# ChalmersPhotonicsLab/QAMpy

Hardware: AMD Instinct MI355X
Metric: equalised MSym/s (2-pol, 2 SPS) (higher is better)
Workload: dtype f32

## Files before the change

### qampy_amd/csrc/train_pit.h

```cpp
#pragma once
#include <atomic>
#include <chrono>
#include <vector>
#include "train_impl.h"
#include "train_seg.h"

namespace qh {

typedef qh_pit_report PitCtrl;

constexpr double PIT_CONTRACT = 0.2;
constexpr int PIT_PROBE = 128;
constexpr int PIT_SEEDWIN = 512;
constexpr int PIT_MAXSEG = 65536;

__host__ __device__ inline int pit_symmetry(int method)
{
    switch (method) {
    case QH_M_CMA: case QH_M_SGNCMA: case QH_M_RDE: return 0;
    case QH_M_CMA2: return 2;
    default: return 4;
    }
}

// ... 763 lines not shown
                        const float c = __builtin_amdgcn_rsqf(1.f + t * t);
                        g = float4{c, t * c, apq.x * rmag, apq.y * rmag};
                    }
                }
                grot[tid] = g; gpair[tid] = ix;
                glog[((size_t)sweep * (m - 1) + r) * npair + tid] = g;
            }
            __syncthreads();
#pragma unroll
            for (int k = 0; k < NB; k++) {
                if (k >= nbt) break;
                const int I = bI[k], J = bJ[k];
                const int2 pi = gpair[I], pj = gpair[J];
                const float4 gi = grot[I], gj = grot[J];
                const bool qi = pi.y < n, qj = pj.y < n;
                const Zf z{0.f, 0.f};
                const Zf a_pr = src[pi.x * ld + pj.x], a_ps = qj ? src[pi.x * ld + pj.y] : z;
                const Zf a_qr = qi ? src[pi.y * ld + pj.x] : z, a_qs = (qi && qj) ? src[pi.y * ld + pj.y] : z;
                const Zf ejc{gj.z, -gj.w};
                const Zf ps_e = cmulf(ejc, a_ps), qs_e = cmulf(ejc, a_qs);
                const Zf t_pr{gj.x * a_pr.x - gj.y * ps_e.x, gj.x * a_pr.y - gj.y * ps_e.y}, t_ps{gj.y * a_pr.x + gj.x * ps_e.x, gj.y * a_pr.y + gj.x * ps_e.y};
                const Zf t_qr{gj.x * a_qr.x - gj.y * qs_e.x, gj.x * a_qr.y - gj.y * qs_e.y}, t_qs{gj.y * a_qr.x + gj.x * qs_e.x, gj.y * a_qr.y + gj.x * qs_e.y};
                const Zf ei{gi.z, gi.w};
                const Zf qr_e = cmulf(ei, t_qr), qs_e2 = cmulf(ei, t_qs);
                const Zf n_pr{gi.x * t_pr.x - gi.y * qr_e.x, gi.x * t_pr.y - gi.y * qr_e.y}, n_ps{gi.x * t_ps.x - gi.y * qs_e2.x, gi.x * t_ps.y - gi.y * qs_e2.y};
                const Zf n_qr{gi.y * t_pr.x + gi.x * qr_e.x, gi.y * t_pr.y + gi.x * qr_e.y}, n_qs{gi.y * t_ps.x + gi.x * qs_e2.x, gi.y * t_ps.y + gi.x * qs_e2.y};
                dst[pi.x * ld + pj.x] = n_pr;
                if (qj) dst[pi.x * ld + pj.y] = n_ps;
                if (qi) dst[pi.y * ld + pj.x] = n_qr;
                if (qi && qj) dst[pi.y * ld + pj.y] = n_qs;
                if (I != J) {
                    dst[pj.x * ld + pi.x] = Zf{n_pr.x, -n_pr.y};
                    if (qj) dst[pj.y * ld + pi.x] = Zf{n_ps.x, -n_ps.y};
                    if (qi) dst[pj.x * ld + pi.y] = Zf{n_qr.x, -n_qr.y};
                    if (qi && qj) dst[pj.y * ld + pi.y] = Zf{n_qs.x, -n_qs.y};
                }
            }
            __syncthreads();
            Zf *t = src; src = dst; dst = t;
        }
    }
    for (int k = tid; k < n; k += 1024) lam[k] = (double)src[k * ld + k].x;
}

constexpr int PIT_JV_CH = 27;
static __global__ void __launch_bounds__(64) pit_jacobi_v_kernel(const float4 *glog, int n, int nsweep, Zf *Vout)
{
    QH_WAVE_FIRST();
    __shared__ Zf row[PIT_EIGMAX + 2];
    __shared__ float4 gch[PIT_JV_CH * (PIT_EIGMAX / 2 + 1)];
    const int lane = threadIdx.x, i = blockIdx.x;
    const int m = (n + 1) & ~1, npair = m / 2;
    for (int k = lane; k < n + 2; k += 64) row[k] = Zf{k == i ? 1.f : 0.f, 0.f};
    const int nround = nsweep * (m - 1);
    for (int r0 = 0; r0 < nround; r0 += PIT_JV_CH) {
        const int nr = nround - r0 < PIT_JV_CH ? nround - r0 : PIT_JV_CH;
        __syncthreads();
        for (int e = lane; e < nr * npair; e += 64) gch[e] = glog[(size_t)r0 * npair + e];
        __syncthreads();
        for (int rr = 0; rr < nr; rr++) {
            const int r = (r0 + rr) % (m - 1);
            if (lane < npair) {
                int pa, pb;
                if (lane == 0) { pa = m - 1; pb = r; }
                else {
                    pa = r + lane; if (pa >= m - 1) pa -= m - 1;
                    pb = r - lane; if (pb < 0) pb += m - 1;
                }
                const int p = pa < pb ? pa : pb, q = pa < pb ? pb : pa;
                if (q < n) {
                    const float4 g = gch[rr * npair + lane];
                    const Zf up = row[p];
                    const Zf xqe = cmulf(Zf{g.z, -g.w}, row[q]);
                    row[p] = Zf{g.x * up.x - g.y * xqe.x, g.x * up.y - g.y * xqe.y};
                    row[q] = Zf{g.y * up.x + g.x * xqe.x, g.y * up.y + g.x * xqe.y};
                }
            }
            __builtin_amdgcn_fence(__ATOMIC_RELEASE, "wavefront");
        }
    }
    for (int k = lane; k < n; k += 64) { Vout[(size_t)i * n + k] = row[k]; Vout[(size_t)n * n + (size_t)k * n + i] = row[k]; }
}

constexpr int PIT_GT = 16, PIT_GC = PIT_GT / 8;
template <typename R> struct PitFuse {
    Cx<R> *X, *Y;
    const double *theta;
    const int64_t *modes_dev;
    int nmodes, nsel;
    float damp = 1.f;
    const Cx<R> *T2 = nullptr;
    float2 *Out2 = nullptr;
};
template <typename R, bool CONJT>
__global__ void __launch_bounds__(256) pit_cgemm_kernel(const Zf *A2, const Zf *B, Zf *C, int n, int ncol, const PitCtrl *c, PitFuse<R> fz)
{
    QH_WAVE_FIRST();
    if (c->done) return;
    extern __shared__ __attribute__((aligned(16))) char pit_smem[];
    Zf *As = reinterpret_cast<Zf *>(pit_smem);
    Zf *Bs = As + (size_t)PIT_EIGMAX * PIT_EIGMAX;
    const int tx = threadIdx.x & 7, ty = threadIdx.x >> 3;
    const int col0 = blockIdx.x * PIT_GT;
    const size_t wset = (size_t)fz.nmodes * n;
    for (int e = threadIdx.x; e < PIT_EIGMAX * n; e += 256) {
        const int k = e / PIT_EIGMAX, m = e - k * PIT_EIGMAX;
        Zf v{0.f, 0.f};
        if (m < n) { v = A2[(size_t)k * n + m]; if (CONJT) v.y = -v.y; }
        As[e] = v;
    }
    if (CONJT) {
        for (int e = threadIdx.x; e < n * PIT_GT; e += 256) {
            const int cc = e / n, k = e - cc * n, col = col0 + cc;
            Zf v{0.f, 0.f};
            if (col < ncol) {
                const int s = col / fz.nsel, j = col - s * fz.nsel;
                if (s > 0) {
                    const size_t ro = (size_t)fz.modes_dev[j] * n;
                    const Cx<R> b = fz.Y[(size_t)(s - 1) * wset + ro + k], a = fz.X[(size_t)s * wset + ro + k];
                    const double pr = fz.theta[2 * (size_t)(col - fz.nsel)], pi = fz.theta[2 * (size_t)(col - fz.nsel) + 1];
                    const double qr = fz.theta[2 * (size_t)col], qi = fz.theta[2 * (size_t)col + 1];
                    v = Zf{(float)((pr * b.re - pi * b.im) - (qr * a.re - qi * a.im)), (float)((pr * b.im + pi * b.re) - (qr * a.im + qi * a.re))};
                }
            }
            Bs[k * PIT_GT + cc] = v;
        }
    } else {
        for (int e = threadIdx.x; e < n * PIT_GT; e += 256) {
            const int k = e / PIT_GT, cc = e - k * PIT_GT;
            Bs[e] = col0 + cc < ncol ? B[(size_t)k * ncol + col0 + cc] : Zf{0.f, 0.f};
        }
    }
    __syncthreads();
    constexpr int RU = PIT_EIGMAX / 32;
    Zf acc[RU][PIT_GC];
#pragma unroll
    for (int u = 0; u < RU; u++)
#pragma unroll
        for (int v = 0; v < PIT_GC; v++) acc[u][v] = Zf{0.f, 0.f};
    for (int k = 0; k < n; k++) {
        Zf b[PIT_GC], a[RU];
#pragma unroll
        for (int v = 0; v < PIT_GC; v++) b[v] = Bs[k * PIT_GT + PIT_GC * tx + v];
#pragma unroll
        for (int u = 0; u < RU; u++) a[u] = As[k * PIT_EIGMAX + ty + 32 * u];
#pragma unroll
        for (int u = 0; u < RU; u++)
#pragma unroll
            for (int v = 0; v < PIT_GC; v++) {
                acc[u][v].x += a[u].x * b[v].x - a[u].y * b[v].y;
                acc[u][v].y += a[u].x * b[v].y + a[u].y * b[v].x;
            }
    }
    if (CONJT) {
#pragma unroll
        for (int u = 0; u < RU; u++) {
            const int m = ty + 32 * u;
            if (m < n)
#pragma unroll
                for (int v = 0; v < PIT_GC; v++)
                    if (col0 + PIT_GC * tx + v < ncol) C[(size_t)m * ncol + col0 + PIT_GC * tx + v] = acc[u][v];
        }
    } else {
#pragma unroll
        for (int v = 0; v < PIT_GC; v++) {
            const int col = col0 + PIT_GC * tx + v;
            if (col >= ncol) continue;
            const int s = col / fz.nsel, j = col - s * fz.nsel;
            const size_t base = (size_t)s * wset + (size_t)fz.modes_dev[j] * n;
            const double qr = fz.theta[2 * (size_t)col], qi = fz.theta[2 * (size_t)col + 1];
#pragma unroll
            for (int u = 0; u < RU; u++) {
                const int m = ty + 32 * u;
                if (m < n) {
                    const Cx<R> x = fz.X[base + m];
// ... 220 lines not shown
        for (int cb = 0; cb < PIT_MC; cb += NCW * nw) {
            Zf tmp[NCW][2];
#pragma unroll
            for (int q = 0; q < NCW; q++) {
                const int cc = cb + wave + nw * q, col = col0 + cc;
                tmp[q][0] = Zf{0.f, 0.f}; tmp[q][1] = Zf{0.f, 0.f};
                if (cc < PIT_MC && col < ncol) {
                    const int s = col / fz.nsel, j = col - s * fz.nsel;
                    const Cx<R> *src = T + (size_t)s * wset + (size_t)fz.modes_dev[j] * n;
                    if (lane < n) { const Cx<R> t = src[lane]; tmp[q][0] = Zf{(float)t.re, (float)t.im}; }
                    if (lane + 64 < n) { const Cx<R> t = src[lane + 64]; tmp[q][1] = Zf{(float)t.re, (float)t.im}; }
                }
            }
#pragma unroll
            for (int q = 0; q < NCW; q++) {
                const int cc = cb + wave + nw * q;
                if (cc < PIT_MC) {
                    if (lane < np) Bs[lane * PIT_MBP + cc] = tmp[q][0];
                    if (lane + 64 < np) Bs[(lane + 64) * PIT_MBP + cc] = tmp[q][1];
                }
            }
        }
    } else {
        const int cc = tid & 15, k0 = tid >> 4, kstep = nt >> 4;
        const bool okc = col0 + cc < ncol;
        for (int kb = 0; kb < np; kb += 8 * kstep) {
            Zf tmp[8];
#pragma unroll
            for (int q = 0; q < 8; q++) {
                const int k = kb + k0 + kstep * q;
                tmp[q] = (okc && k < n) ? D[(size_t)k * ncol + col0 + cc] : Zf{0.f, 0.f};
            }
#pragma unroll
            for (int q = 0; q < 8; q++) {
                const int k = kb + k0 + kstep * q;
                if (k < np) Bs[k * PIT_MBP + cc] = tmp[q];
            }
        }
    }
    const bool pre = MODE == 1 && NCW * nw >= PIT_MC;
    Cx<R> xv[MODE == 1 ? NCW : 1][2];
    double th[MODE == 1 ? NCW : 1][2];
    if (pre) {
#pragma unroll
        for (int q = 0; q < NCW; q++) {
            const int cc = wave + nw * q, col = col0 + cc;
            xv[q][0] = Cx<R>{0, 0}; xv[q][1] = Cx<R>{0, 0}; th[q][0] = 1; th[q][1] = 0;
            if (cc < PIT_MC && col < ncol) {
                const int s = col / fz.nsel, j = col - s * fz.nsel;
                const size_t base = (size_t)s * wset + (size_t)fz.modes_dev[j] * n;
                th[q][0] = fz.theta[2 * (size_t)col]; th[q][1] = fz.theta[2 * (size_t)col + 1];
                if (lane < n) xv[q][0] = fz.X[base + lane];
                if (lane + 64 < n) xv[q][1] = fz.X[base + lane + 64];
            }
        }
    }
    __syncthreads();
    pit_f4 rr = {0.f, 0.f, 0.f, 0.f}, ii = rr, im = rr;
    const Zf *bp = Bs + (lane >> 4) * PIT_MBP + (lane & 15);
    for (int k0 = 0; k0 < np; k0 += 4 * PF) {
#pragma unroll
        for (int i = 0; i < PF; i++) {
            const int k = k0 + 4 * i;
            if (k < np) {
                Zf a = abuf[i];
                abuf[i] = lda(k + 4 * PF);
                if (MODE == 0) a.y = -a.y;
                const Zf b = bp[(size_t)k * PIT_MBP];
                rr = __builtin_amdgcn_mfma_f32_16x16x4f32(a.x, b.x, rr, 0, 0, 0);
                ii = __builtin_amdgcn_mfma_f32_16x16x4f32(a.y, b.y, ii, 0, 0, 0);
                im = __builtin_amdgcn_mfma_f32_16x16x4f32(a.x, b.y, im, 0, 0, 0);
                im = __builtin_amdgcn_mfma_f32_16x16x4f32(a.y, b.x, im, 0, 0, 0);
            }
        }
    }
    const int cl = lane & 15;
    if (MODE == 0) {
        const int col = col0 + cl;
#pragma unroll
        for (int q = 0; q < 4; q++) {
            const int m = 16 * wave + 4 * (lane >> 4) + q;
            if (m < n && col < ncol) Out[(size_t)m * ncol + col] = Zf{rr[q] - ii[q], im[q]};
        }
    } else {
#pragma unroll
        for (int q = 0; q < 4; q++) {
            const int m = 16 * wave + 4 * (lane >> 4) + q;
            Ct[cl * (PIT_EIGMAX + 1) + m] = Zf{rr[q] - ii[q], im[q]};
        }
        __syncthreads();
        for (int cb = 0; cb < PIT_MC; cb += NCW * nw) {
#pragma unroll
            for (int q = 0; q < NCW; q++) {
                const int cc = cb + wave + nw * q, col = col0 + cc;
                if (cc < PIT_MC && col < ncol) {
                    const int s = col / fz.nsel, j = col - s * fz.nsel;
                    const size_t base = (size_t)s * wset + (size_t)fz.modes_dev[j] * n;
                    const double qr = pre ? th[q][0] : fz.theta[2 * (size_t)col], qi = pre ? th[q][1] : fz.theta[2 * (size_t)col + 1];
#pragma unroll
                    for (int h = 0; h < 2; h++) {
                        const int m = lane + 64 * h;
                        if (m < n) {
                            const Cx<R> x = pre ? xv[q][h] : fz.X[base + m];
                            const Zf d = Ct[cc * (PIT_EIGMAX + 1) + m];
                            const Cx<R> w{(R)(qr * x.re - qi * x.im + fz.damp * d.x), (R)(qr * x.im + qi * x.re + fz.damp * d.y)};
                            fz.X[base + m] = w;
                            fz.Y[base + m] = w;
                        }
                    }
                }
            }
        }
    }
}

static __global__ void __launch_bounds__(256) pit_bound_kernel(const Zf *Xe, const Zf *Ye, const Zf *Yprev, const double *lam, int n, int S, int nsel, int sym,
                                                              const PitCtrl *c, double *dfc, double *pw, double *gph, float4 *ualpha = nullptr)
{
    QH_WAVE_FIRST();
    if (c->done) return;
    const int lane = threadIdx.x & 63, bi = blockIdx.x * 4 + (threadIdx.x >> 6);
    const int nb = (S - 1) * nsel, ncol = S * nsel;
    if (bi >= nb + nsel) return;
    const bool result_probe = bi >= nb;
    const int j = result_probe ? bi - nb : bi % nsel;
    const int sb = result_probe ? S - 1 : bi / nsel;
    const Zf *pa = result_probe ? (c->passes == 0 ? Xe + (size_t)(S - 1) * nsel + j : Yprev + j) : Xe + (size_t)(sb + 1) * nsel + j;
    const size_t sa = (result_probe && c->passes != 0) ? (size_t)nsel : (size_t)ncol;
    const Zf *pb = Ye + (size_t)sb * nsel + j;
    Zf av[(PIT_EIGMAX + 63) / 64], bv[(PIT_EIGMAX + 63) / 64];
    float lv[(PIT_EIGMAX + 63) / 64];
    double A = 0, B = 0, Cr = 0, Ci = 0;
#pragma unroll
    for (int q = 0; q < (PIT_EIGMAX + 63) / 64; q++) {
        const int k = lane + 64 * q;
        av[q] = Zf{0.f, 0.f}; bv[q] = Zf{0.f, 0.f}; lv[q] = 0.f;
        if (k < n) {
            av[q] = pa[(size_t)k * sa]; bv[q] = pb[(size_t)k * ncol];
            const float l = (float)lam[k];
            lv[q] = l > 0.f ? l : 0.f;
        }
        A += (double)lv[q] * ((double)av[q].x * av[q].x + (double)av[q].y * av[q].y);
        B += (double)lv[q] * ((double)bv[q].x * bv[q].x + (double)bv[q].y * bv[q].y);
        Cr += (double)lv[q] * ((double)bv[q].x * av[q].x + (double)bv[q].y * av[q].y);
        Ci += (double)lv[q] * ((double)bv[q].y * av[q].x - (double)bv[q].x * av[q].y);
    }
    for (int o = 32; o > 0; o >>= 1) { A += __shfl_xor(A, o); B += __shfl_xor(B, o); Cr += __shfl_xor(Cr, o); Ci += __shfl_xor(Ci, o); }
    double gr = 1, gi = 0;
    if (sym == 0) {
        const double pr = sqrt(Cr * Cr + Ci * Ci);
        if (pr > 0) { gr = Cr / pr; gi = Ci / pr; }
    } else if (sym == 4 || sym == 2 || sym == 1) {
        if (sym == 4 && fabs(Ci) > fabs(Cr)) { gr = 0; gi = Ci >= 0 ? 1 : -1; }
        else if (sym == 1) gr = 1;
        else gr = Cr >= 0 ? 1 : -1;
    } else {
        const double step = 6.283185307179586 / sym;
        const double kk = rint(atan2(Ci, Cr) / step) * step;
        gr = cos(kk); gi = sin(kk);
    }
    double d2 = 0;
    const float grf = (float)gr, gif = (float)gi;
#pragma unroll
    for (int q = 0; q < (PIT_EIGMAX + 63) / 64; q++) {
        const float dr = bv[q].x - (grf * av[q].x - gif * av[q].y), di = bv[q].y - (grf * av[q].y + gif * av[q].x);
        d2 += (double)lv[q] * ((double)dr * dr + (double)di * di);
    }
    for (int o = 32; o > 0; o >>= 1) d2 += __shfl_xor(d2, o);
    if (ualpha && !result_probe) {
        float nn = 0.f, ar = 0.f, ai = 0.f;
#pragma unroll
        for (int q = 0; q < (PIT_EIGMAX + 63) / 64; q++) {
            const float dr = bv[q].x - (grf * av[q].x - gif * av[q].y), di = bv[q].y - (grf * av[q].y + gif * av[q].x);
            const float ur = lv[q] * bv[q].x, ui = lv[q] * bv[q].y;
            nn += ur * ur + ui * ui;
            ar += ur * dr + ui * di;
            ai += ur * di - ui * dr;
        }
        for (int o = 32; o > 0; o >>= 1) { nn += __shfl_xor(nn, o); ar += __shfl_xor(ar, o); ai += __shfl_xor(ai, o); }
        const float inv = nn > 0.f ? rsqrtf(nn) : 0.f;
        if (lane == 0) ualpha[bi] = float4{ar * inv, ai * inv, inv, 0.f};
    }
    if (lane == 0) {
        if (!result_probe) { gph[2 * (size_t)bi] = gr; gph[2 * (size_t)bi + 1] = gi; pw[bi] = B; }
        dfc[bi] = (A == A && B == B) ? sqrt(d2 / (B > 1e-300 ? B : 1e-300)) : 1e30;
    }
}

constexpr int PIT_RT = 1024;
template <typename R>
__global__ void __launch_bounds__(PIT_RT) pit_recur_eig_kernel(Zf *Xe, const Zf *Ye, Zf *D, const double *theta, const double *lam, int nsel, int S, int64_t T, const R *mu,
                                                               double beta, const PitCtrl *c, const float *Msum = nullptr, float damp = 1.f,
                                                               const float4 *ualpha = nullptr, const float2 *uq = nullptr)
{
    QH_WAVE_FIRST();
    if (c->done) return;
    __shared__ float4 aff[2 * PIT_RT];
    const int k = blockIdx.x, j = blockIdx.y;
    const int ncol = S * nsel;
    Zf *row = D + (size_t)k * ncol + j, *xr = Xe + (size_t)k * ncol + j;
    const Zf *yr = Ye + (size_t)k * ncol + j;
    double a = (double)*mu * c->gain * (double)T * lam[k];
    if (a < 0) a = 0;
    const float coef = c->corr_on ? (float)exp(-a * (1 + beta * a)) : 0.f;
    const float gl = (float)(c->gain * lam[k] > 0 ? c->gain * lam[k] : 0.0), betaf = (float)beta;
    const bool corr = c->corr_on != 0;
    auto cf = [&](int s) -> float {
        if (!Msum) return coef;
        const float as = gl * Msum[(size_t)s * nsel + j];
        return corr ? __expf(-as * (1.f + betaf * as)) : 0.f;
    };
    const int len = (S + PIT_RT - 1) / PIT_RT;
    const int s0 = threadIdx.x * len, s1 = s0 + len < S ? s0 + len : S;
    auto th = [&](int s) { return Zf{(float)theta[2 * ((size_t)s * nsel + j)], (float)theta[2 * ((size_t)s * nsel + j) + 1]}; };
    auto scan_op = [](float4 e, float4 l) { return float4{l.x * e.x, l.x * e.y + l.y, l.x * e.z + l.z, 0.f}; };
    if (len <= 4) {
        Zf y[4], x[4], t[5], r[4];
        t[0] = s0 > 0 && s0 < S ? th(s0 - 1) : Zf{1.f, 0.f};
#pragma unroll
        for (int q = 0; q < 4; q++) {
            const int s = s0 + q;
            const bool ok = s < s1;
            y[q] = (ok && s > 0) ? yr[(size_t)(s - 1) * nsel] : Zf{0.f, 0.f};
            x[q] = ok ? xr[(size_t)s * nsel] : Zf{0.f, 0.f};
            t[q + 1] = ok ? th(s) : Zf{1.f, 0.f};
        }
        Zf run{0.f, 0.f};
        float cq[4], clen = 1.f;
        float4 ua[4];
        float2 qq[4];
        const float lk = (float)(lam[k] > 0 ? lam[k] : 0.0);
#pragma unroll
        for (int q = 0; q < 4; q++) {
            const int s = s0 + q;
            cq[q] = (s < s1 && s > 0) ? cf(s - 1) : (s < s1 ? 0.f : 1.f);
            ua[q] = (ualpha && s < s1 && s > 0) ? ualpha[(size_t)(s - 1) * nsel + j] : float4{0.f, 0.f, 0.f, 0.f};
            qq[q] = (uq && s < s1 && s > 0) ? uq[(size_t)s * nsel + j] : float2{0.f, 0.f};
        }
        Zf uk[4];
#pragma unroll
        for (int q = 0; q < 4; q++) {
            const int s = s0 + q;
            uk[q] = Zf{0.f, 0.f};
            if (s < s1) {
                x[q] = cmulf(t[q + 1], x[q]);
                Zf d{0.f, 0.f};
                if (s > 0) {
                    const Zf aa = cmulf(t[q], y[q]);
                    d = Zf{aa.x - x[q].x, aa.y - x[q].y};
                    uk[q] = Zf{aa.x * lk * ua[q].z, aa.y * lk * ua[q].z};
                    const Zf ual = cmulf(uk[q], Zf{ua[q].x, ua[q].y});
                    d = Zf{d.x - ual.x, d.y - ual.y};
                }
                run = Zf{d.x + cq[q] * run.x, d.y + cq[q] * run.y};
                r[q] = run;
                clen *= cq[q];
            }
        }
        const float4 comp = block_scan_excl<float4, decltype(scan_op), PIT_RT>(float4{clen, run.x, run.y, 0.f}, scan_op, float4{1.f, 0.f, 0.f, 0.f}, aff);
        float pw = 1.f;
#pragma unroll
        for (int q = 0; q < 4; q++) {
            const int s = s0 + q;
            if (s < s1) {
                pw *= cq[q];
                const Zf uqv = cmulf(uk[q], Zf{qq[q].x, qq[q].y});
                const Zf v{r[q].x + pw * comp.y + uqv.x, r[q].y + pw * comp.z + uqv.y};
                row[(size_t)s * nsel] = v;
// ... 629 lines not shown
        if (exact_only) {
            QH_REQUIRE(!o.exchange, "train_equaliser: a capture split over processes needs the parallel-in-time solver (blind / decision-directed method, fixed step)");
            void *cb0 = nullptr;
            if ((rc = scratch(8, sizeof(PitCtrl) + 64, &cb0))) return rc;
            PitCtrl *c0 = report_dev ? (PitCtrl *)report_dev : (PitCtrl *)cb0;
            PitSeg s1; s1.S = 1; s1.len = TrSyms; s1.extra = 0; s1.tail = 0;
            hipLaunchKernelGGL((pit_setup_kernel<R>), dim3(1), dim3(256), 0, g_stream, (const Cx<R> *)E, nmodes, L, (int64_t)(L < 4096 ? L : 4096), nmodes * ntaps, (const R *)mu_dev, 1.0, 1.0,
                               o.tol > 0 ? o.tol : 1e-3, s1, c0, (R *)((char *)cb0 + sizeof(PitCtrl)));
            return exact_form(c0, o.adaptive, zero_err, adaptive ? nullptr : gram, 0);
        }
    }
    if (adaptive) o.acquire = 0;
    const int ntot = nmodes * ntaps;
    const int npass = o.max_passes > 0 ? o.max_passes : (adaptive ? QH_PIT_MAXPASS : 16);
    const double tol = (o.tol > 0 ? o.tol : 1e-3) * (adaptive ? 1.0 / 3.0 : 1.0);
    const double safety = o.dev_safety > 0 ? o.dev_safety : PIT_DEV_SAFETY;
    const int sym = pit_symmetry(method);
    const bool seed_phase = o.phase_seed < 0 ? sym == 4 : o.phase_seed != 0;
    const bool want_corr = o.correction != 0 && pit_basis_ok(ntot, sizeof(Cx<R>));
    double beta = o.corr_beta >= 0 ? o.corr_beta : (sym == 0 ? 1.5 : 0.0);

    void *cbuf = nullptr;
    if ((rc = scratch(8, sizeof(PitCtrl) + 64, &cbuf))) return rc;
    PitCtrl *ctrl = report_dev ? (PitCtrl *)report_dev : (PitCtrl *)cbuf;
    R *mu_acq = (R *)((char *)cbuf + sizeof(PitCtrl));

    int S = o.segments;
    const float ad_relax = 1.0f, ad_damp = 0.7f;
    const int ad_newton = 1;
    const int64_t head_want = 16384;
    int64_t head = adaptive ? ((TrSyms / 4 < head_want ? TrSyms / 4 : head_want) / LA_B * LA_B) : 0;
    if (!adaptive && o.head_steps > 0) {
        QH_REQUIRE(!o.exchange, "train_equaliser: a capture split over processes takes no exact head");
        head = (int64_t)o.head_steps / LA_B * LA_B;
        if (head > TrSyms) head = TrSyms / LA_B * LA_B;
        o.acquire = 0;
    }
    int64_t seg_want = 2048;
    if (adaptive && !(method == QH_M_SBD || method == QH_M_MDDMA || method == QH_M_DD)) {
        const int64_t t = ((TrSyms - head) / 512 + LA_B - 1) / LA_B * LA_B;
        if (t > seg_want) seg_want = t;
    }
    if (S == 0 && adaptive) S = (int)((TrSyms - head) / seg_want < PIT_MAXSEG ? (TrSyms - head) / seg_want : PIT_MAXSEG);
    if (S == 0) {
        R mu_h = (R)o.mu_hint;
        if (!(o.mu_hint > 0)) {
            QH_HIP(hipMemcpyAsync(&mu_h, mu_dev, sizeof(R), hipMemcpyDeviceToHost, g_stream));
            QH_HIP(hipStreamSynchronize(g_stream));
        }
        S = pit_auto_segments(TrSyms, (double)mu_h, nsel, o.acquire);
    }
    PitPlan pl = pit_plan(o, TrSyms, head, S, adaptive, o.acquire ? o.acq_chunk : 0);
    const PitSeg &sg = pl.sg;
    if (zero_err) QH_HIP(hipMemsetAsync(err, 0, (size_t)nmodes * TrSyms * Niter * sizeof(Cx<R>), g_stream));
    const int64_t npow = L < 4096 ? L : 4096;
    hipLaunchKernelGGL((pit_setup_kernel<R>), dim3(1), dim3(256), 0, g_stream, (const Cx<R> *)E, nmodes, L, npow, ntot, (const R *)mu_dev, pl.gear, pl.bound, tol, sg, ctrl, mu_acq);
    QH_HIP(hipGetLastError());
    if (TrSyms == 0 || Niter == 0) return QH_OK;
    if (sg.S < 2) {
        const double zero = 0;
        QH_HIP(hipMemcpyAsync(&ctrl->defect[0], &zero, sizeof(double), hipMemcpyHostToDevice, g_stream));
        return exact_form(ctrl, adaptive ? 1 : 0, 0, gram, 1);
    }

    TrainerForm f;
    if ((rc = trainer_form<R>(f, FORM_PASSES, method, adaptive, nmodes, ntaps, os, sg.len, (int64_t)sg.S * nsel, symbols, nsy, modes, nsel))) return rc;
    if (adaptive && !f.seg) return exact_form(ctrl, 1, 0, nullptr, 0);
    const bool decision = method == QH_M_SBD || method == QH_M_MDDMA || method == QH_M_DD;
    const bool seg_form = f.seg, use_bi = f.use_bi, block_form = f.block, pair_tab = f.pair_tab;
    const bool split = o.exchange != nullptr;
    const int own_first = split ? o.seg_first : 0, own_count = split ? o.seg_count : sg.S;
    const bool xchg_async = split && o.exchange_on_stream != 0;
    if (split) {
        QH_REQUIRE(seg_form, "train_equaliser: a capture split over processes needs the throughput form of the passes (>= 512 chains, supported tap layout)");
        QH_REQUIRE(own_first >= 0 && own_count >= 0 && own_first + own_count <= sg.S, "train_equaliser: owned segments outside the segment grid");
        QH_REQUIRE(Niter == 1, "train_equaliser: a capture split over processes is trained in one sweep");
    }

    const size_t wset = (size_t)nmodes * ntot;
    const size_t wbytes = wset * sizeof(Cx<R>);
    void *wbuf = nullptr;
    const size_t nsj = (size_t)sg.S * nsel;
    const size_t bytes_w = ((2 * (size_t)sg.S + 2) * wbytes + 63) / 64 * 64;
    if ((rc = scratch(2, bytes_w + 10 * nsj * sizeof(double) + (size_t)nsel * sizeof(int64_t) + 320 + nsj * 16 + 4 * ((nsj + 63) / 64) * sizeof(float) + 64, &wbuf))) return rc;
    Cx<R> *X = (Cx<R> *)wbuf, *Y = X + (size_t)sg.S * wset, *w_start = Y + (size_t)sg.S * wset, *w_call = w_start + wset;
    double *z = (double *)((char *)wbuf + bytes_w), *rot = z + 2 * nsj, *dfc = rot + 2 * nsj, *pw = dfc + nsj, *gph = pw + nsj, *theta = gph + 2 * nsj;
    int64_t *modes_dev = (int64_t *)(theta + 2 * nsj);
    double *uw_phi = (double *)(modes_dev + ((nsel + 7) / 8 * 8));
    int *uw_jump = (int *)(uw_phi + (size_t)sg.S * nsel);
    float *devmax = (float *)(uw_jump + (size_t)sg.S * nsel);
    const int ndev = (int)((nsj + 63) / 64);
    unsigned *ticket = (unsigned *)(devmax + 4 * (size_t)ndev);
    PitInit init{};
    init.z[0] = ticket; init.zn[0] = sizeof(unsigned);
    R *ad_rS = nullptr, *ad_rE = nullptr;
    Cx<R> *ad_eS = nullptr, *ad_eE = nullptr, *ad_errh = nullptr;
    float *ad_M = nullptr, *ad_chg = nullptr, *ad_rP = nullptr, *ad_dP = nullptr;
    if (!adaptive && head > 0) {
        void *ab = nullptr;
        if ((rc = scratch(13, (size_t)nmodes * head * sizeof(Cx<R>) + 64, &ab))) return rc;
        ad_errh = (Cx<R> *)ab;
    }
    if (adaptive) {
        void *ab = nullptr;
        const size_t nS = ((size_t)sg.S + 15) / 16 * 16;
        if ((rc = scratch(13, nS * (2 * sizeof(R) + 2 * sizeof(Cx<R>) + 3 * sizeof(float)) + 64 + (size_t)nmodes * head * sizeof(Cx<R>), &ab))) return rc;
        ad_eS = (Cx<R> *)ab; ad_eE = ad_eS + nS; ad_errh = ad_eE + nS;
        ad_rS = (R *)(ad_errh + (size_t)nmodes * head); ad_rE = ad_rS + nS;
        ad_M = (float *)(ad_rE + nS); ad_rP = ad_M + nS; ad_dP = ad_rP + nS; ad_chg = ad_dP + nS;
    }
    init.modes_dev = modes_dev; init.nsel = nsel;
    for (int j = 0; j < 16; j++) init.modes[j] = j < nsel ? modes[j] : 0;
    const bool prepared = o.prepared != nullptr && o.acquire && !adaptive && head == 0 && Niter >= 1;
    const bool need_mu = adaptive || !(o.mu_hint > 0), need_acq = o.acquire && !(o.acq_chunk > 0) && !prepared;
    R mu_acq_h = 0;
    if (need_acq) QH_HIP(hipMemcpyAsync(&mu_acq_h, mu_acq, sizeof(R), hipMemcpyDeviceToHost, g_stream));
    R mu_host = need_mu ? (R)1 : (R)o.mu_hint;
    if (need_mu) QH_HIP(hipMemcpyAsync(&mu_host, mu_dev, sizeof(R), hipMemcpyDeviceToHost, g_stream));
    if (need_mu || need_acq) QH_HIP(hipStreamSynchronize(g_stream));
    if (!adaptive && !(mu_host != 0))
        return exact_form(ctrl, 0, 0, gram, 0);
    if (o.acquire && !(o.acq_chunk > 0)) pl.acquisition(o, TrSyms, pit_acq_chunk(mu_acq_h));

    const int64_t amax = pl.amax;
    void *G = const_cast<void *>(gram);
    if (prepared) QH_REQUIRE(seg_form && o.acq_chunk > 0, "train_equaliser: a prepared acquisition belongs to throughput-form passes with acq_chunk given (qh_pit_prepare_*_dev said so)");
    if (block_form && !G && (!seg_form || amax > 0) && !prepared) {
        const int64_t n = seg_form ? pl.ngram : TrSyms;
        rc = pair_tab ? gram_build<R>(E, nmodes, L, os, ntaps, n, &G) : gram_cur_build<R>(E, nmodes, L, os, ntaps, n, &G);
        if (rc) return rc;
    }
    const int64_t g_per_step = pair_tab ? LA_B : GRAM_TRI / 2 / LA_B;

    const int ncol = sg.S * nsel;
    const double *lam = nullptr;
    const Zf *Vb = nullptr;
    Zf *Dz[2] = {nullptr, nullptr};
    Zf *Xe = nullptr, *Ye = nullptr, *Yprev = nullptr;
    if (want_corr) {
        void *cb = nullptr;
        if ((rc = scratch(10, pit_basis_bytes(ntot) + 4 * (size_t)ntot * ncol * sizeof(Zf) + (size_t)ntot * nsel * sizeof(Zf) + 256, &cb))) return rc;
        void *basis = o.basis ? o.basis : cb;
        if (!o.basis && (rc = pit_basis<R>(E, nmodes, L, os, ntaps, TrSyms, basis))) return rc;
        lam = (const double *)basis; Vb = (const Zf *)((const char *)basis + (size_t)ntot * sizeof(double));
        Dz[0] = (Zf *)((char *)cb + (pit_basis_bytes(ntot) + 63) / 64 * 64); Dz[1] = Dz[0] + (size_t)ntot * ncol;
        Xe = Dz[1] + (size_t)ntot * ncol; Ye = Xe + (size_t)ntot * ncol; Yprev = Ye + (size_t)ntot * ncol;
    }
    const bool eig = want_corr && sizeof(R) == 4 && form(FORM_PIT_PROBE) == 0;
    const bool tables_ok = method == QH_M_CMA || method == QH_M_SGNCMA || method == QH_M_MCMA || method == QH_M_RDE || method == QH_M_MRDE ||
                           (decision && (use_bi || seg_form));
    const bool ssb = eig && tables_ok && method != QH_M_CMA2;
    PitModel *model = nullptr;
    float4 *ualpha = nullptr;
    float2 *uqv = nullptr;
    PitModelArgs<R> ma;
    hipEvent_t model_event = nullptr;
    if (ssb) {
        void *mb = nullptr;
        const size_t pw_ = 2 * PIT_EIGMAX + 8;
        const size_t b_part = (size_t)PIT_MODB * 4 * nsel * pw_ * sizeof(float), b_u = ((size_t)nsel * ntot * sizeof(Cx<R>) + 63) / 64 * 64;
        const size_t b_ua = ((size_t)ncol * sizeof(float4) + 63) / 64 * 64, b_uq = ((size_t)ncol * sizeof(float2) + 63) / 64 * 64;
        if ((rc = scratch(14, b_part + b_u + b_ua + b_uq + 16 * sizeof(PitModel) + 128, &mb))) return rc;
        ma.part = (float *)mb; ma.u = (Cx<R> *)((char *)mb + b_part);
        ualpha = (float4 *)((char *)mb + b_part + b_u); uqv = (float2 *)((char *)ualpha + b_ua);
        model = (PitModel *)((char *)uqv + b_uq); ma.model = model; ma.ticket = (unsigned *)(model + 16);
        init.z[1] = ma.ticket; init.zn[1] = sizeof(unsigned);
        init.z[2] = ualpha; init.zn[2] = (unsigned)(b_ua + b_uq);
        ma.E = (const Cx<R> *)E; ma.wx = (const Cx<R> *)wx; ma.L = L; ma.TrSyms = TrSyms; ma.nmodes = nmodes; ma.ntaps = ntaps; ma.os = os; ma.nsel = nsel; ma.method = method;
        if (decision) { ma.symbols = (const Cx<R> *)f.dd_table; ma.nsy = 2 * f.dd_npart + 1; ma.sy_pitch = 2 * BI_DD_MAXLEV; ma.tables = 1; }
        else { ma.symbols = (const Cx<R> *)symbols; ma.nsy = nsy; ma.sy_pitch = nsy; ma.tables = (method == QH_M_RDE || method == QH_M_MRDE) ? 1 : 0; }
        for (int j = 0; j < 16; j++) ma.modes[j] = j < nsel ? modes[j] : 0;
        if (o.corr_beta < 0) beta = 0.0;
    }
    const size_t glds = ((size_t)PIT_EIGMAX * PIT_EIGMAX + (size_t)PIT_EIGMAX * PIT_GT) * sizeof(Zf);
    static std::atomic<bool> gemm_attr{false};
    if (want_corr && !gemm_attr.load(std::memory_order_acquire)) {
        QH_HIP(hipFuncSetAttribute((const void *)pit_cgemm_kernel<R, true>, hipFuncAttributeMaxDynamicSharedMemorySize, 160 * 1024 - 256));
// ... 73 lines not shown
            hipLaunchKernelGGL((pit_model_kernel<R, 0>), dim3(PIT_MODB), dim3(256), 0, ss, ma);
            hipLaunchKernelGGL((pit_model_kernel<R, 1>), dim3(PIT_MODB), dim3(256), 0, ss, ma);
            QH_HIP(hipEventRecord(ev_model, ss));
            model_event = ev_model;
        }
        QH_HIP(hipGetLastError());
        const int timing_mode = pit_timing_mode();
        auto decide_args = [&](int p, const float *dm, const float2 *ye, float2 *yprev, int ne, int ncol_e, int corr_wanted) {
            PitDecideArgs<R> d;
            d.dfc = dfc; d.pw = pw; d.nb = (int)((sg.S - 1) * nsel); d.Ylast = (const Cx<R> *)(Y + (size_t)(sg.S - 1) * wset); d.n = (int)wset; d.wx = (Cx<R> *)wx; d.c = ctrl;
            d.host_view = &ev.hview[2 * p]; d.nrow = nsel; d.devmax = dm; d.ndev = ndev; d.safety = safety; d.Ye = ye; d.Yprev = yprev; d.ne = ne; d.ncol_e = ncol_e;
            d.theta = theta; d.modes_dev = (const int64_t *)modes_dev; d.ntot_w = ntot; d.S = (int)sg.S; d.sym = sym; d.corr_wanted = corr_wanted;
            d.extra = adaptive ? (const float *)ad_chg : nullptr;
            d.Dfin = (ye && !adaptive) ? (const float2 *)Dz[1] : nullptr; d.Vfin = (const float2 *)Vb; d.lam_fin = lam;
            d.stall_from = adaptive ? 5 : 2;
            return d;
        };
        auto timed = [&](int p) { return timing_mode == 2 || (timing_mode == 1 && p == 1); };
        auto enqueue_pass = [&](int p) -> int {
            ((volatile float *)ev.hview)[2 * p] = -1.f;
            PitFuse<R> fz;
            fz.X = X; fz.Y = Y; fz.theta = theta; fz.modes_dev = (const int64_t *)modes_dev; fz.nmodes = nmodes; fz.nsel = nsel;
            fz.damp = (adaptive && p > 1) ? ad_damp : 1.f;
            if (p > 0 && want_corr) {
                if (eig)
                    hipLaunchKernelGGL((pit_basis_mfma_kernel<R, 1>), dim3((ncol + PIT_MC - 1) / PIT_MC), dim3(pit_mfma_threads(ntot)), pit_mfma_lds(ntot), g_stream, Vb + (size_t)ntot * ntot,
                                       (const Cx<R> *)nullptr, (const Zf *)Dz[1], (Zf *)nullptr, ntot, ncol, (const PitCtrl *)ctrl, fz);
                else
                    hipLaunchKernelGGL((pit_cgemm_kernel<R, false>), dim3((ncol + PIT_GT - 1) / PIT_GT), dim3(256), glds, g_stream, Vb + (size_t)ntot * ntot, (const Zf *)Dz[1], (Zf *)nullptr, ntot, ncol, (const PitCtrl *)ctrl, fz);
                QH_HIP(hipGetLastError());
            } else if (p > 0) {
                QH_HIP(hipMemcpyAsync(X + wset, Y, (size_t)(sg.S - 1) * wbytes, hipMemcpyDeviceToDevice, g_stream));
                QH_HIP(hipMemcpyAsync(Y, X, (size_t)sg.S * wbytes, hipMemcpyDeviceToDevice, g_stream));
            }
            if (o.on_pass) {
                hipStream_t keep = g_stream;
                o.on_pass(o.on_pass_user, it, p);
                g_stream = keep;
            }
            if (timed(p)) QH_HIP(hipEventRecord(ev.t0[p], g_stream));
            if (seg_form) {
                SegArgs<R> sa{};
                sa.E = (const Cx<R> *)E; sa.wx = Y; sa.symbols = la.symbols; sa.err = (Cx<R> *)err; sa.mu = mu_dev;
                sa.L = L; sa.TrSyms = TrSyms; sa.nsy = la.nsy; sa.sy_pitch = la.sy_pitch; sa.err_pitch = TrSyms * Niter; sa.err_off = (int64_t)it * TrSyms;
                sa.nmodes = nmodes; sa.ntaps = ntaps; sa.os = os; sa.nsel = nsel; sa.S = sg.S;
                sa.seg_len = sg.len; sa.seg_extra = sg.extra; sa.seg_tail = sg.tail; sa.seg_begin = sg.begin;
                sa.r_in = ad_rS; sa.r_out = ad_rE; sa.e_in = ad_eS; sa.e_out = ad_eE; sa.mu_sum = (R *)ad_M; sa.adapt_first = sg.begin > 0 ? 1 : 0;
                for (int j = 0; j < 16; j++) sa.modes[j] = j < nsel ? modes[j] : 0;
                sa.skip = &ctrl->done;
                sa.q_first = own_first * nsel; sa.q_count = split ? own_count * nsel : 0;
                if (!split || own_count > 0) { int r = launch_seg<R>(sa, method, adaptive); if (r) return r; }
                if (adaptive) hipLaunchKernelGGL((pit_adapt_scan_kernel<R>), dim3(1), dim3(1024), 0, g_stream, ad_rS, (const R *)ad_rE, ad_eS, (const Cx<R> *)ad_eE, sg.S, ad_chg, (const PitCtrl *)ctrl, ad_relax, ad_rP, ad_dP, ad_newton);
            } else if (block_form) {
                LaArgs<R> ls = la;
                ls.TrSyms = sg.len; ls.nch = sg.S; ls.wx = Y; ls.err_off = (int64_t)it * TrSyms; ls.seg = 1; ls.seg_extra = sg.extra; ls.seg_tail = sg.tail;
                ls.skip = &ctrl->done;
                if (sg.begin > 0) {
                    ls.E = (const Cx<R> *)E + sg.begin * os; ls.L = L - sg.begin * os; ls.err_off += sg.begin;
                    ls.G = (const GramPair<R> *)G + sg.begin * g_per_step;
                }
                { int r = use_bi ? launch_bi<R>(ls) : launch_la<R>(ls); if (r) return r; }
            } else {
                TrainArgs<R> ts = ta;
                ts.wx = Y; ts.nseg = sg.S; ts.seg_begin = sg.begin; ts.seg_len = sg.len; ts.seg_extra = sg.extra; ts.seg_tail = sg.tail; ts.seg_iter = it; ts.skip = &ctrl->done;
                { int r = launch_any<R>(ts); if (r) return r; }
            }
            if (timed(p)) QH_HIP(hipEventRecord(ev.t1[p], g_stream));
            if (split) {
                if (own_first > 0) QH_HIP(hipMemsetAsync(Y, 0, (size_t)own_first * wbytes, g_stream));
                if (own_first + own_count < sg.S)
                    QH_HIP(hipMemsetAsync(Y + (size_t)(own_first + own_count) * wset, 0, (size_t)(sg.S - own_first - own_count) * wbytes, g_stream));
                if (!xchg_async) QH_HIP(hipStreamSynchronize(g_stream));
                if (o.exchange(o.exchange_user, Y, (size_t)sg.S * wbytes) != 0) { set_error("train_equaliser: the exchange callback failed"); return QH_ERR_ARG; }
            }
            const int nbnd = (int)((sg.S - 1) * nsel);
            if (eig) {
                if (o.basis && pit_basis_sync().pending) {
                    QH_HIP(hipStreamWaitEvent(g_stream, pit_basis_sync().out, 0));
                    pit_basis_sync().pending = false;
                }
                auto forward2 = [&](const Cx<R> *src, Zf *dst, const Cx<R> *src2, Zf *dst2) {
                    PitFuse<R> f2 = fz;
                    f2.T2 = src2; f2.Out2 = reinterpret_cast<float2 *>(dst2);
                    hipLaunchKernelGGL((pit_basis_mfma_kernel<R, 0>), dim3(2 * ((ncol + PIT_MC - 1) / PIT_MC)), dim3(pit_mfma_threads(ntot)), pit_mfma_lds(ntot), g_stream, Vb, src, (const Zf *)nullptr, dst, ntot, ncol, (const PitCtrl *)ctrl, f2);
                };
                if (p == 0 && model_event) QH_HIP(hipStreamWaitEvent(g_stream, model_event, 0));
                forward2((const Cx<R> *)X, Xe, (const Cx<R> *)Y, Ye);
                hipLaunchKernelGGL(pit_bound_kernel, dim3((nbnd + nsel + 3) / 4), dim3(256), 0, g_stream, (const Zf *)Xe, (const Zf *)Ye, (const Zf *)Yprev, lam, ntot, sg.S, nsel, sym,
                                   (const PitCtrl *)ctrl, dfc, pw, gph, ualpha);
                hipLaunchKernelGGL((pit_gauge_kernel<R>), dim3(ssb ? 2 : 1), dim3(PIT_GT_THREADS), 0, g_stream, (const double *)gph, sg.S, nsel, ctrl, theta, (const double *)pw,
                                   nbnd, method, (const Cx<R> *)symbols + (size_t)modes[0] * nsy, 1, (const PitModel *)model, (const float4 *)ualpha, uqv,
                                   (const R *)mu_dev, sg.len, (const float *)ad_M);
                hipLaunchKernelGGL((pit_recur_eig_kernel<R>), dim3(ntot, nsel), dim3(PIT_RT), 0, g_stream, Xe, (const Zf *)Ye, Dz[1], (const double *)theta, lam, nsel, sg.S, sg.len,
                                   (const R *)mu_dev, beta, (const PitCtrl *)ctrl, (const float *)ad_M, (adaptive && p >= 1) ? ad_damp : 1.f,
                                   (const float4 *)ualpha, (const float2 *)uqv);
                hipLaunchKernelGGL((pit_devest_kernel<R>), dim3(ndev), dim3(256), 0, g_stream, (const Zf *)Dz[1], lam, ntot, ncol, (const PitCtrl *)ctrl, devmax, ticket,
                                   decide_args(p, (const float *)devmax, (const float2 *)Ye, (float2 *)Yprev, ntot, ncol, 1));
            } else {
            const size_t dlds = (2 * (size_t)ntot + (size_t)nmodes * os * pit_phase_pitch(ntaps, os, PIT_PROBE)) * sizeof(Cx<R>);
            QH_REQUIRE(dlds <= 60 * 1024, "train_equaliser: boundary probe does not fit the LDS for this filter shape");
            hipLaunchKernelGGL((pit_defect_kernel<R>), dim3(sg.S, nsel), dim3(PIT_PROBE), dlds, g_stream, (const Cx<R> *)E, nmodes, L, os,
                               ntaps, sg, TrSyms, (const int64_t *)modes_dev, (const Cx<R> *)X, (const Cx<R> *)Y, sym, (const PitCtrl *)ctrl, dfc, pw, gph, (const Cx<R> *)wx);
            hipLaunchKernelGGL((pit_gauge_kernel<R>), dim3(1), dim3(PIT_GT_THREADS), 0, g_stream, (const double *)gph, sg.S, nsel, ctrl, theta, (const double *)pw,
                               nbnd, method, (const Cx<R> *)symbols + (size_t)modes[0] * nsy, want_corr ? 1 : 0);
            if (want_corr) {
                if (o.basis && pit_basis_sync().pending) {
                    QH_HIP(hipStreamWaitEvent(g_stream, pit_basis_sync().out, 0));
                    pit_basis_sync().pending = false;
                }
                hipLaunchKernelGGL((pit_cgemm_kernel<R, true>), dim3((ncol + PIT_GT - 1) / PIT_GT), dim3(256), glds, g_stream, Vb, (const Zf *)nullptr, Dz[1], ntot, ncol, (const PitCtrl *)ctrl, fz);
                hipLaunchKernelGGL((pit_recur_kernel<R>), dim3(ntot, nsel), dim3(256), 0, g_stream, Dz[1], lam, nsel, sg.S, sg.len, (const R *)mu_dev, beta, (const PitCtrl *)ctrl);
                hipLaunchKernelGGL((pit_devest_kernel<R>), dim3(ndev), dim3(256), 0, g_stream, (const Zf *)Dz[1], lam, ntot, ncol, (const PitCtrl *)ctrl, devmax, ticket,
                                   decide_args(p, (const float *)devmax, (const float2 *)nullptr, (float2 *)nullptr, 0, 0, 1));
            } else
                hipLaunchKernelGGL((pit_decide_kernel<R>), dim3(1), dim3(256), 0, g_stream, decide_args(p, (const float *)nullptr, (const float2 *)nullptr, (float2 *)nullptr, 0, 0, 0));
            }
            QH_HIP(hipGetLastError());
            return QH_OK;
        };
        if ((rc = enqueue_pass(0))) return rc;
        if (it == 0 && o.on_pass0) {
            hipStream_t keep = g_stream;
            o.on_pass0(o.on_pass0_user);
            g_stream = keep;
        }
        bool ahead = false;
        bool certified = false;
        for (int p = 0; p < npass; p++) {
            double contr = PIT_CONTRACT;
            if (p >= 2 && ev.hview[2 * (p - 2) + 1] > 0) {
                contr = (double)ev.hview[2 * (p - 1) + 1] / (double)ev.hview[2 * (p - 2) + 1];
                contr = contr < 0.1 ? 0.1 : (contr > 0.9 ? 0.9 : contr);
            }
            const bool expect_last = p > 0 && contr * (double)ev.hview[2 * (p - 1) + 1] < tol;
            ahead = false;
            if (p + 1 < npass && !expect_last && (!split || xchg_async)) { if ((rc = enqueue_pass(p + 1))) return rc; ahead = true; }
            {
                volatile float *hv = (volatile float *)ev.hview;
                unsigned spins = 0;
                auto t_last = std::chrono::steady_clock::now();
                while (hv[2 * p] < 0.f) {
                    if ((++spins & 255u) != 0) continue;
                    const auto now = std::chrono::steady_clock::now();
                    if (now - t_last < std::chrono::milliseconds(20)) continue;
                    t_last = now;
                    const hipError_t q = hipStreamQuery(g_stream);
                    if (q == hipSuccess) { if (hv[2 * p] < 0.f) hv[2 * p] = 2.f; break; }
                    if (q != hipErrorNotReady) QH_HIP(q);
                }
                std::atomic_thread_fence(std::memory_order_acquire);
            }
            if (timed(p) && tm.npass < QH_PIT_MAXPASS) {
                float ms = 0;
                QH_HIP(hipEventSynchronize(ev.t1[p]));
                QH_HIP(hipEventElapsedTime(&ms, ev.t0[p], ev.t1[p]));
                tm.pass_ms[tm.npass++] = ms;
            }
            if (ev.hview[2 * p] != 0.f) { certified = ev.hview[2 * p] == 1.f; break; }
            if (p + 1 < npass && !ahead && (rc = enqueue_pass(p + 1))) return rc;
        }
        if (acq_timed) {
            float ms = 0;
            QH_HIP(hipEventSynchronize(ev.t1[PIT_NEV - 1]));
            QH_HIP(hipEventElapsedTime(&ms, ev.t0[PIT_NEV - 1], ev.t1[PIT_NEV - 1]));
            tm.acq_ms = ms; acq_timed = false;
        }
        if (!adaptive && !certified && redo_ok && !split && depth < 3 && o.head_auto_off == 0) {
            double hp = 0;
            int hfront[2] = {-1, 0};
            bool finite = false;
            if (eig) {
                int *fr = (int *)(ticket + 4);
// ... 103 lines not shown
```

Baseline: 1202.

## Fuse boundary-probe reduction into basis MFMA kernel via per-tile tickets

Removes the separate pit_bound_kernel launch and runs the boundary/defect reduction inside the forward basis MFMA kernel. The last block to finish the tiles a boundary needs, found through atomic tile tickets, computes those boundaries. This is meant to save a kernel launch and a pass over Xe/Ye that may still be in cache. The cost is threadfences, atomics and extra tail work in some blocks, plus a correctness risk from the ticket ordering and from resetting tickets across passes.

Measured after the change: 949.1. -21.0%, worse.

```diff
diff --git a/qampy_amd/csrc/train_pit.h b/qampy_amd/csrc/train_pit.h
--- a/qampy_amd/csrc/train_pit.h
+++ b/qampy_amd/csrc/train_pit.h
@@ -869,6 +869,88 @@
     for (int k = lane; k < n; k += 64) { Vout[(size_t)i * n + k] = row[k]; Vout[(size_t)n * n + (size_t)k * n + i] = row[k]; }
 }
 
+struct PitBound {
+    const Zf *Xe, *Ye, *Yprev;
+    const double *lam;
+    double *dfc, *pw, *gph;
+    float4 *ualpha;
+    unsigned *tile_ticket = nullptr;
+    int S, sym;
+};
+__device__ __forceinline__ void pit_bound_wave(const PitBound &bd, int n, int nsel, const PitCtrl *c, int bi, int lane)
+{
+    const Zf *Xe = bd.Xe, *Ye = bd.Ye, *Yprev = bd.Yprev;
+    const double *lam = bd.lam;
+    double *dfc = bd.dfc, *pw = bd.pw, *gph = bd.gph;
+    float4 *ualpha = bd.ualpha;
+    const int S = bd.S, sym = bd.sym;
+    const int nb = (S - 1) * nsel, ncol = S * nsel;
+    const bool result_probe = bi >= nb;
+    const int j = result_probe ? bi - nb : bi % nsel;
+    const int sb = result_probe ? S - 1 : bi / nsel;
+    const Zf *pa = result_probe ? (c->passes == 0 ? Xe + (size_t)(S - 1) * nsel + j : Yprev + j) : Xe + (size_t)(sb + 1) * nsel + j;
+    const size_t sa = (result_probe && c->passes != 0) ? (size_t)nsel : (size_t)ncol;
+    const Zf *pb = Ye + (size_t)sb * nsel + j;
+    Zf av[(PIT_EIGMAX + 63) / 64], bv[(PIT_EIGMAX + 63) / 64];
+    float lv[(PIT_EIGMAX + 63) / 64];
+    double A = 0, B = 0, Cr = 0, Ci = 0;
+#pragma unroll
+    for (int q = 0; q < (PIT_EIGMAX + 63) / 64; q++) {
+        const int k = lane + 64 * q;
+        av[q] = Zf{0.f, 0.f}; bv[q] = Zf{0.f, 0.f}; lv[q] = 0.f;
+        if (k < n) {
+            av[q] = pa[(size_t)k * sa]; bv[q] = pb[(size_t)k * ncol];
+            const float l = (float)lam[k];
+            lv[q] = l > 0.f ? l : 0.f;
+        }
+        A += (double)lv[q] * ((double)av[q].x * av[q].x + (double)av[q].y * av[q].y);
+        B += (double)lv[q] * ((double)bv[q].x * bv[q].x + (double)bv[q].y * bv[q].y);
+        Cr += (double)lv[q] * ((double)bv[q].x * av[q].x + (double)bv[q].y * av[q].y);
+        Ci += (double)lv[q] * ((double)bv[q].y * av[q].x - (double)bv[q].x * av[q].y);
+    }
+    for (int o = 32; o > 0; o >>= 1) { A += __shfl_xor(A, o); B += __shfl_xor(B, o); Cr += __shfl_xor(Cr, o); Ci += __shfl_xor(Ci, o); }
+    double gr = 1, gi = 0;
+    if (sym == 0) {
+        const double pr = sqrt(Cr * Cr + Ci * Ci);
+        if (pr > 0) { gr = Cr / pr; gi = Ci / pr; }
+    } else if (sym == 4 || sym == 2 || sym == 1) {
+        if (sym == 4 && fabs(Ci) > fabs(Cr)) { gr = 0; gi = Ci >= 0 ? 1 : -1; }
+        else if (sym == 1) gr = 1;
+        else gr = Cr >= 0 ? 1 : -1;
+    } else {
+        const double step = 6.283185307179586 / sym;
+        const double kk = rint(atan2(Ci, Cr) / step) * step;
+        gr = cos(kk); gi = sin(kk);
+    }
+    double d2 = 0;
+    const float grf = (float)gr, gif = (float)gi;
+#pragma unroll
+    for (int q = 0; q < (PIT_EIGMAX + 63) / 64; q++) {
+        const float dr = bv[q].x - (grf * av[q].x - gif * av[q].y), di = bv[q].y - (grf * av[q].y + gif * av[q].x);
+        d2 += (double)lv[q] * ((double)dr * dr + (double)di * di);
+    }
+    for (int o = 32; o > 0; o >>= 1) d2 += __shfl_xor(d2, o);
+    if (ualpha && !result_probe) {
+        float nn = 0.f, ar = 0.f, ai = 0.f;
+#pragma unroll
+        for (int q = 0; q < (PIT_EIGMAX + 63) / 64; q++) {
+            const float dr = bv[q].x - (grf * av[q].x - gif * av[q].y), di = bv[q].y - (grf * av[q].y + gif * av[q].x);
+            const float ur = lv[q] * bv[q].x, ui = lv[q] * bv[q].y;
+            nn += ur * ur + ui * ui;
+            ar += ur * dr + ui * di;
+            ai += ur * di - ui * dr;
+        }
+        for (int o = 32; o > 0; o >>= 1) { nn += __shfl_xor(nn, o); ar += __shfl_xor(ar, o); ai += __shfl_xor(ai, o); }
+        const float inv = nn > 0.f ? rsqrtf(nn) : 0.f;
+        if (lane == 0) ualpha[bi] = float4{ar * inv, ai * inv, inv, 0.f};
+    }
+    if (lane == 0) {
+        if (!result_probe) { gph[2 * (size_t)bi] = gr; gph[2 * (size_t)bi + 1] = gi; pw[bi] = B; }
+        dfc[bi] = (A == A && B == B) ? sqrt(d2 / (B > 1e-300 ? B : 1e-300)) : 1e30;
+    }
+}
+
+
 constexpr int PIT_GT = 16, PIT_GC = PIT_GT / 8;
 template <typename R> struct PitFuse {
     Cx<R> *X, *Y;
@@ -878,6 +960,7 @@
     float damp = 1.f;
     const Cx<R> *T2 = nullptr;
     float2 *Out2 = nullptr;
+    PitBound bd{};
 };
 template <typename R, bool CONJT>
 __global__ void __launch_bounds__(256) pit_cgemm_kernel(const Zf *A2, const Zf *B, Zf *C, int n, int ncol, const PitCtrl *c, PitFuse<R> fz)
@@ -1264,6 +1347,30 @@
             const int m = 16 * wave + 4 * (lane >> 4) + q;
             if (m < n && col < ncol) Out[(size_t)m * ncol + col] = Zf{rr[q] - ii[q], im[q]};
         }
+        if (fz.bd.tile_ticket) {
+            __shared__ int mine[2];
+            const int t = col0 / PIT_MC;
+            __threadfence();
+            __syncthreads();
+            if (tid == 0) {
+                unsigned *tk = fz.bd.tile_ticket;
+                int w0 = -1, w1 = -1;
+                if (atomicAdd(&tk[t], 1u) == (t + 1 < nb1 ? 2u : 1u)) { tk[t] = 0; w0 = t; }
+                if (!second && t > 0 && atomicAdd(&tk[t - 1], 1u) == 2u) { tk[t - 1] = 0; w1 = t - 1; }
+                mine[0] = w0; mine[1] = w1;
+            }
+            __syncthreads();
+#pragma unroll
+            for (int e = 0; e < 2; e++) {
+                const int tile = mine[e];
+                if (tile < 0) continue;
+                __threadfence();
+                for (int bq = wave; bq < PIT_MC; bq += nw) {
+                    const int bi = tile * PIT_MC + bq;
+                    if (bi < ncol) pit_bound_wave(fz.bd, n, fz.nsel, c, bi, lane);
+                }
+            }
+        }
     } else {
 #pragma unroll
         for (int q = 0; q < 4; q++) {
@@ -1293,79 +1400,6 @@
                 }
             }
         }
-    }
-}
-
-static __global__ void __launch_bounds__(256) pit_bound_kernel(const Zf *Xe, const Zf *Ye, const Zf *Yprev, const double *lam, int n, int S, int nsel, int sym,
-                                                              const PitCtrl *c, double *dfc, double *pw, double *gph, float4 *ualpha = nullptr)
-{
-    QH_WAVE_FIRST();
-    if (c->done) return;
-    const int lane = threadIdx.x & 63, bi = blockIdx.x * 4 + (threadIdx.x >> 6);
-    const int nb = (S - 1) * nsel, ncol = S * nsel;
-    if (bi >= nb + nsel) return;
-    const bool result_probe = bi >= nb;
-    const int j = result_probe ? bi - nb : bi % nsel;
-    const int sb = result_probe ? S - 1 : bi / nsel;
-    const Zf *pa = result_probe ? (c->passes == 0 ? Xe + (size_t)(S - 1) * nsel + j : Yprev + j) : Xe + (size_t)(sb + 1) * nsel + j;
-    const size_t sa = (result_probe && c->passes != 0) ? (size_t)nsel : (size_t)ncol;
-    const Zf *pb = Ye + (size_t)sb * nsel + j;
-    Zf av[(PIT_EIGMAX + 63) / 64], bv[(PIT_EIGMAX + 63) / 64];
-    float lv[(PIT_EIGMAX + 63) / 64];
-    double A = 0, B = 0, Cr = 0, Ci = 0;
-#pragma unroll
-    for (int q = 0; q < (PIT_EIGMAX + 63) / 64; q++) {
-        const int k = lane + 64 * q;
-        av[q] = Zf{0.f, 0.f}; bv[q] = Zf{0.f, 0.f}; lv[q] = 0.f;
-        if (k < n) {
-            av[q] = pa[(size_t)k * sa]; bv[q] = pb[(size_t)k * ncol];
-            const float l = (float)lam[k];
-            lv[q] = l > 0.f ? l : 0.f;
-        }
-        A += (double)lv[q] * ((double)av[q].x * av[q].x + (double)av[q].y * av[q].y);
-        B += (double)lv[q] * ((double)bv[q].x * bv[q].x + (double)bv[q].y * bv[q].y);
-        Cr += (double)lv[q] * ((double)bv[q].x * av[q].x + (double)bv[q].y * av[q].y);
-        Ci += (double)lv[q] * ((double)bv[q].y * av[q].x - (double)bv[q].x * av[q].y);
-    }
-    for (int o = 32; o > 0; o >>= 1) { A += __shfl_xor(A, o); B += __shfl_xor(B, o); Cr += __shfl_xor(Cr, o); Ci += __shfl_xor(Ci, o); }
-    double gr = 1, gi = 0;
-    if (sym == 0) {
-        const double pr = sqrt(Cr * Cr + Ci * Ci);
-        if (pr > 0) { gr = Cr / pr; gi = Ci / pr; }
-    } else if (sym == 4 || sym == 2 || sym == 1) {
-        if (sym == 4 && fabs(Ci) > fabs(Cr)) { gr = 0; gi = Ci >= 0 ? 1 : -1; }
-        else if (sym == 1) gr = 1;
-        else gr = Cr >= 0 ? 1 : -1;
-    } else {
-        const double step = 6.283185307179586 / sym;
-        const double kk = rint(atan2(Ci, Cr) / step) * step;
-        gr = cos(kk); gi = sin(kk);
-    }
-    double d2 = 0;
-    const float grf = (float)gr, gif = (float)gi;
-#pragma unroll
-    for (int q = 0; q < (PIT_EIGMAX + 63) / 64; q++) {
-        const float dr = bv[q].x - (grf * av[q].x - gif * av[q].y), di = bv[q].y - (grf * av[q].y + gif * av[q].x);
-        d2 += (double)lv[q] * ((double)dr * dr + (double)di * di);
-    }
-    for (int o = 32; o > 0; o >>= 1) d2 += __shfl_xor(d2, o);
-    if (ualpha && !result_probe) {
-        float nn = 0.f, ar = 0.f, ai = 0.f;
-#pragma unroll
-        for (int q = 0; q < (PIT_EIGMAX + 63) / 64; q++) {
-            const float dr = bv[q].x - (grf * av[q].x - gif * av[q].y), di = bv[q].y - (grf * av[q].y + gif * av[q].x);
-            const float ur = lv[q] * bv[q].x, ui = lv[q] * bv[q].y;
-            nn += ur * ur + ui * ui;
-            ar += ur * dr + ui * di;
-            ai += ur * di - ui * dr;
-        }
-        for (int o = 32; o > 0; o >>= 1) { nn += __shfl_xor(nn, o); ar += __shfl_xor(ar, o); ai += __shfl_xor(ai, o); }
-        const float inv = nn > 0.f ? rsqrtf(nn) : 0.f;
-        if (lane == 0) ualpha[bi] = float4{ar * inv, ai * inv, inv, 0.f};
-    }
-    if (lane == 0) {
-        if (!result_probe) { gph[2 * (size_t)bi] = gr; gph[2 * (size_t)bi + 1] = gi; pw[bi] = B; }
-        dfc[bi] = (A == A && B == B) ? sqrt(d2 / (B > 1e-300 ? B : 1e-300)) : 1e30;
     }
 }
 
@@ -2161,7 +2195,7 @@
     void *wbuf = nullptr;
     const size_t nsj = (size_t)sg.S * nsel;
     const size_t bytes_w = ((2 * (size_t)sg.S + 2) * wbytes + 63) / 64 * 64;
-    if ((rc = scratch(2, bytes_w + 10 * nsj * sizeof(double) + (size_t)nsel * sizeof(int64_t) + 320 + nsj * 16 + 4 * ((nsj + 63) / 64) * sizeof(float) + 64, &wbuf))) return rc;
+    if ((rc = scratch(2, bytes_w + 10 * nsj * sizeof(double) + (size_t)nsel * sizeof(int64_t) + 320 + nsj * 16 + 4 * ((nsj + 63) / 64) * sizeof(float) + (8 + (nsj + 15) / 16) * sizeof(unsigned) + 64, &wbuf))) return rc;
     Cx<R> *X = (Cx<R> *)wbuf, *Y = X + (size_t)sg.S * wset, *w_start = Y + (size_t)sg.S * wset, *w_call = w_start + wset;
     double *z = (double *)((char *)wbuf + bytes_w), *rot = z + 2 * nsj, *dfc = rot + 2 * nsj, *pw = dfc + nsj, *gph = pw + nsj, *theta = gph + 2 * nsj;
     int64_t *modes_dev = (int64_t *)(theta + 2 * nsj);
@@ -2171,7 +2205,8 @@
     const int ndev = (int)((nsj + 63) / 64);
     unsigned *ticket = (unsigned *)(devmax + 4 * (size_t)ndev);
     PitInit init{};
-    init.z[0] = ticket; init.zn[0] = sizeof(unsigned);
+    unsigned *tile_ticket = ticket + 8;
+    init.z[0] = ticket; init.zn[0] = (unsigned)((8 + (nsj + 15) / 16) * sizeof(unsigned));
     R *ad_rS = nullptr, *ad_rE = nullptr;
     Cx<R> *ad_eS = nullptr, *ad_eE = nullptr, *ad_errh = nullptr;
     float *ad_M = nullptr, *ad_chg = nullptr, *ad_rP = nullptr, *ad_dP = nullptr;
@@ -2411,12 +2446,12 @@
                 auto forward2 = [&](const Cx<R> *src, Zf *dst, const Cx<R> *src2, Zf *dst2) {
                     PitFuse<R> f2 = fz;
                     f2.T2 = src2; f2.Out2 = reinterpret_cast<float2 *>(dst2);
+                    f2.bd.Xe = dst; f2.bd.Ye = dst2; f2.bd.Yprev = Yprev; f2.bd.lam = lam; f2.bd.dfc = dfc; f2.bd.pw = pw; f2.bd.gph = gph; f2.bd.ualpha = ualpha;
+                    f2.bd.tile_ticket = tile_ticket; f2.bd.S = (int)sg.S; f2.bd.sym = sym;
                     hipLaunchKernelGGL((pit_basis_mfma_kernel<R, 0>), dim3(2 * ((ncol + PIT_MC - 1) / PIT_MC)), dim3(pit_mfma_threads(ntot)), pit_mfma_lds(ntot), g_stream, Vb, src, (const Zf *)nullptr, dst, ntot, ncol, (const PitCtrl *)ctrl, f2);
                 };
                 if (p == 0 && model_event) QH_HIP(hipStreamWaitEvent(g_stream, model_event, 0));
                 forward2((const Cx<R> *)X, Xe, (const Cx<R> *)Y, Ye);
-                hipLaunchKernelGGL(pit_bound_kernel, dim3((nbnd + nsel + 3) / 4), dim3(256), 0, g_stream, (const Zf *)Xe, (const Zf *)Ye, (const Zf *)Yprev, lam, ntot, sg.S, nsel, sym,
-                                   (const PitCtrl *)ctrl, dfc, pw, gph, ualpha);
                 hipLaunchKernelGGL((pit_gauge_kernel<R>), dim3(ssb ? 2 : 1), dim3(PIT_GT_THREADS), 0, g_stream, (const double *)gph, sg.S, nsel, ctrl, theta, (const double *)pw,
                                    nbnd, method, (const Cx<R> *)symbols + (size_t)modes[0] * nsy, 1, (const PitModel *)model, (const float4 *)ualpha, uqv,
                                    (const R *)mu_dev, sg.len, (const float *)ad_M);
```
